# wadewilliamsw1234/Multi-level-Indoor-SLAM

Measured on AMD Instinct MI355X. Metric: keyframes gated/sec (VPR+kNN+LightGlue verify), higher is better.
Workload: dtype bf16

## Files before the change

include/mlgate.h:

```cpp
#ifndef MLGATE_H
#define MLGATE_H

#include <stddef.h>
#include <stdint.h>

#ifdef __cplusplus
extern "C" {
#endif

#define MLG_OK 0
#define MLG_EINVAL (-1)
#define MLG_EHIP (-2)
#define MLG_ENOMEM (-3)

#define MLG_VIT_DEPTH 12
#define MLG_VIT_EMBED 768
#define MLG_VIT_PATCH_K 768

#define MLG_ABI_VERSION 3
#define MLG_STRUCT_INIT(T) {(uint32_t)sizeof(T), (uint32_t)MLG_ABI_VERSION}
int mlg_abi_version(void);
const char* mlg_strerror(int status);

typedef struct mlg_vit_block {
    const float *norm1_w, *norm1_b;
    const uint16_t* qkv_w;
    const float* qkv_b;
    const uint16_t* proj_w;
    const float *proj_b, *ls1;
    const float *norm2_w, *norm2_b;
    const uint16_t* fc1_w;
    const float* fc1_b;
    const uint16_t* fc2_w;
    const float *fc2_b, *ls2;
} mlg_vit_block;

typedef struct mlg_vit_weights {
    uint32_t struct_size, abi_version;
    const uint16_t* patch_w;
    const float* patch_b;
    const float* cls;
    const float* pos;
    mlg_vit_block blocks[MLG_VIT_DEPTH];
    const float *norm_w, *norm_b;
    int packing;
} mlg_vit_weights;

#define MLG_VIT_POOL_MEAN 1
#define MLG_VIT_KEEP_CHANNELS 2
#define MLG_VIT_SPLIT 4

size_t mlg_vit_workspace_bytes(int batch, int image_size);

int mlg_vit_forward(const mlg_vit_weights* w, const uint8_t* frames, int batch, int H, int W, int C,
                    long frame_stride, int image_size, int flags, void* workspace, size_t workspace_bytes,
                    float* desc_out, float* local_out, void* stream);

typedef struct mlg_salad_weights {
    uint32_t struct_size, abi_version;
    const uint16_t* w1;
    const float* b1;
    const uint16_t* w2;
    const float* b2;
    const float *wt1, *bt1, *wt2, *bt2;
    float dust_bin;
} mlg_salad_weights;

#define MLG_SALAD_DIM 8448

size_t mlg_salad_workspace_bytes(int batch, int image_size);

int mlg_salad_forward(const mlg_vit_weights* w, const mlg_salad_weights* sw, const uint8_t* frames, int batch,
                      int H, int W, int C, long frame_stride, int image_size, void* workspace,
                      size_t workspace_bytes, float* desc_out, void* stream);

size_t mlg_knn_workspace_bytes(int N, int D, int Q);
size_t mlg_knn_workspace_bytes_k(int N, int D, int Q, int k, int query);
int mlg_knn_gate(const float* desc, int N, int D, const double* t, const int64_t* floor, const uint8_t* has_floor,
                 double min_gap, float thr, int k, int gating, int q0, int Q, void* workspace,
                 size_t workspace_bytes, int32_t* idx, float* sim, uint8_t* valid, int32_t* count,
                 unsigned long long* totals, void* stream);

int mlg_knn_query(const float* db, int N, int D, const float* qdesc, int Q, const double* t_db,
                  const double* t_query, double min_gap, int k, void* workspace, size_t workspace_bytes,
                  int32_t* idx, float* sim, int32_t* count, void* stream);

int mlg_row_normalize_f32(const float* X, float* Xn, int N, int D, float* norms_or_null, void* stream);
int mlg_similarity(const float* A, int Q, const float* B, int N, int D, float* S, void* stream);

size_t mlg_xcorr_workspace_bytes(int n1, int n2, int D);
int mlg_xcorr_score(const float* q, int n1, const float* m, int n2, int D, void* workspace, size_t workspace_bytes,
                    float* score, void* stream);

size_t mlg_xcorr_batch_workspace_bytes(int F, int L, int D, int P);
int mlg_xcorr_batch(const float* feats, int F, int L, int D, const int32_t* query, const int32_t* cand, int P,
                    void* workspace, size_t workspace_bytes, float* scores, void* stream);

int mlg_op_gemm_f32out(const uint16_t* A, const uint16_t* W, float* C, int M, int N, int K, void* stream);
int mlg_set_gemm_variant(int variant);
int mlg_op_gemm_f32out_variant(int variant, const uint16_t* A, const uint16_t* W, float* C, int M, int N, int K,
                               void* stream);
int mlg_op_gemm_bias_gelu(const uint16_t* A, const uint16_t* W, const float* bias, uint16_t* C, int M, int N,
                          int K, void* stream);
int mlg_op_gemm_residual(const uint16_t* A, const uint16_t* W, const float* bias, const float* gamma, float* X,
                         int M, int N, int K, void* stream);
int mlg_op_layernorm_bf16(const float* X, const float* g, const float* b, uint16_t* Y, int M, void* stream);
int mlg_op_attention(const uint16_t* Q, const uint16_t* K, const uint16_t* Vt, uint16_t* O, int B, int T, int Tpad,
                     int32_t* task_ws, void* stream);
int mlg_op_attention_varlen(const uint16_t* Q, const uint16_t* K, const uint16_t* Vt, uint16_t* O, int ldo, int Npad,
                            int heads, const int32_t* tasks, const int32_t* out_off, int ntasks, int max_q,
                            void* stream);
int mlg_op_lg_ffn(const uint16_t* ctx, float* X, uint16_t* xcopy, int ldc, int M, const uint16_t* Wout,
                  const float* bout, const uint16_t* Wf1, const float* bf1, const float* ln_g, const float* ln_b,
                  const uint16_t* Wf2, const float* bf2, void* stream);
int mlg_op_lg_proj(int self_block, const uint16_t* xcopy, int ldx, const uint16_t* W, const float* bias,
                   const float* ecos, const float* esin, const uint8_t* live, uint16_t* Q, uint16_t* K, uint16_t* Vt,
                   int Npad, void* stream);
int mlg_op_conv2d_nhwc(const uint16_t* in, const uint16_t* zero16, int B, int H, int W, int C, int k, int s,
                       const uint16_t* Wt, const float* bias, float* out, int N, void* stream);
int mlg_op_preprocess_patches(const uint8_t* frames, int B, int H, int W, int C, long frame_stride, int S,
                              uint16_t* patches, void* stream);

size_t mlg_plane_ransac_workspace_bytes(int S, int iterations);
int mlg_plane_ransac(const float* pts, const int32_t* offsets, int S, int iterations, uint64_t seed, double threshold,
                     void* workspace, size_t workspace_bytes, double* plane, double* ratio, int32_t* inliers,
                     void* stream);

size_t mlg_proximity_workspace_bytes(int N, int nrows);
int mlg_proximity_count(const double* pos, const int64_t* floor, int N, int row0, int nrows, double radius,
                        int min_gap, int strict, void* workspace, size_t workspace_bytes, long long* totals,
                        void* stream);
int mlg_proximity_emit(const double* pos, const int64_t* floor, int N, int row0, int nrows, double radius,
                       int min_gap, int strict, const void* workspace, size_t workspace_bytes, int32_t* pairs,
                       double* dist, uint8_t* valid, void* stream);

typedef struct mlg_rn_block {
    const uint16_t* w1; const float* b1;
    const uint16_t* w2; const float* b2;
    const uint16_t* w3; const float* b3;
    const uint16_t* wd; const float* bd;
} mlg_rn_block;
typedef struct mlg_rn_weights {
    uint32_t struct_size, abi_version;
    const float* stem_w;
    const float* stem_b;
    mlg_rn_block blocks[16];
} mlg_rn_weights;
size_t mlg_resnet50_workspace_bytes(int B, int H, int W);
int mlg_resnet50_forward(const mlg_rn_weights* w, const uint8_t* frames, int B, int H, int W, int C,
                         long frame_stride, int descriptor_dim, void* workspace, size_t workspace_bytes,
                         float* desc, void* stream);
int mlg_op_pillow_resize_224(const uint8_t* frames, int B, int H, int W, int C, long frame_stride, void* workspace,
                             size_t workspace_bytes, uint8_t* out, void* stream);

typedef struct mlg_mixvpr_weights {
    uint32_t struct_size, abi_version;
    const float* stem_w;
    const float* stem_b;
    mlg_rn_block blocks[13];
    const uint16_t* mix_w;
    const float* mix_p;
    const float* row_w;
    const float* chan_w;
    const float* chan_b;
    const float* row_s;
    const float* row_b;
} mlg_mixvpr_weights;
#define MLG_MIXVPR_DIM 4096
#define MLG_MIXVPR_SIZE 320
size_t mlg_mixvpr_workspace_bytes(int B, int H, int W);
int mlg_mixvpr_forward(const mlg_mixvpr_weights* w, const uint8_t* frames, int B, int H, int W, int C,
                       long frame_stride, void* workspace, size_t workspace_bytes, float* desc, void* stream);
int mlg_op_mixvpr_preprocess(const uint8_t* frames, int B, int H, int W, int C, long frame_stride, float* out,
                             void* stream);
int mlg_op_mixvpr_head(const mlg_mixvpr_weights* w, const float* features, int B, float* desc, void* stream);

typedef struct mlg_sp_weights {
    uint32_t struct_size, abi_version;
    const float* conv1a_w;
    const float* conv1a_b;
    const uint16_t* w[11];
    const float* b[11];
} mlg_sp_weights;
size_t mlg_superpoint_workspace_bytes(int B, int H, int W);
int mlg_superpoint(const mlg_sp_weights* w, const uint8_t* frames, int B, int H, int W, int C, long frame_stride,
                   float detection_threshold, int max_keypoints, int nms_radius, int remove_borders, void* workspace,
                   size_t workspace_bytes, float* keypoints, float* scores, float* descriptors,
                   uint16_t* descriptors_bf16, int32_t* counts, void* stream);
// ... 146 lines not shown
```

multi-level-indoor-slam_amd/csrc/abi.cpp:

```cpp
#include <hip/hip_runtime.h>

#include <math.h>

#include <mutex>
#include <vector>

#include "../../include/mlgate.h"
#include <cstddef>

#include "kernels.h"

namespace {

constexpr int PATCH = 14;

inline size_t align_up(size_t v, size_t a = 256) { return (v + a - 1) / a * a; }

struct VitGeom {
    int B, S, grid, P, T, Tpad;
    explicit VitGeom(int b, int s) : B(b), S(s), grid(s / PATCH), P(grid * grid), T(grid * grid + 1) {
        Tpad = (T + 63) / 64 * 64;
    }
};

// ... 452 lines not shown
size_t mlg_superglue_workspace_bytes(int P, int kmax) { return mlg_superglue_ws_bytes(P, kmax); }

int mlg_superglue(const mlg_sg_weights* w, const float* keypoints, const float* scores, const float* descriptors,
                  const int32_t* counts, int F, int kmax, int W, int H, const int32_t* pair_a, const int32_t* pair_b,
                  int P, int sinkhorn_iterations, float match_threshold, void* workspace, size_t workspace_bytes,
                  int32_t* matches, float* match_scores, int32_t* num_matches, void* stream) {
    if (!mlg_head_ok(w, MLG_ABI_VERSION) || !keypoints || !scores || !descriptors || !counts || !pair_a || !pair_b ||
        !workspace || !matches || !match_scores || !num_matches || F <= 0 || P <= 0 || W <= 0 || H <= 0)
        return MLG_EINVAL;
    for (int p = 0; p < P; ++p)
        if (pair_a[p] < 0 || pair_a[p] >= F || pair_b[p] < 0 || pair_b[p] >= F) return MLG_EINVAL;
    const mlg_sg_weights_i& wi = *reinterpret_cast<const mlg_sg_weights_i*>(&w->kenc_w);
    return mlg_superglue_run(wi, keypoints, scores, descriptors, counts, kmax, W, H, pair_a, pair_b, P,
                             sinkhorn_iterations, match_threshold, workspace, workspace_bytes, matches, match_scores,
                             num_matches, (hipStream_t)stream);
}

size_t mlg_ransac_workspace_bytes(int P, long S_total, int hypotheses) {
    return mlg_ransac_ws_bytes(P, S_total, hypotheses);
}

int mlg_ransac_epipolar(const float* kp1, const float* kp2, const int32_t* offsets, int P, long S_total,
                        const double* K, int k_stride, double threshold, int hypotheses, uint64_t seed,
                        void* workspace, size_t workspace_bytes, double* model, uint8_t* mask, int32_t* inliers,
                        double* pose, int32_t* status, void* stream) {
    if (!offsets || !workspace || !model || !inliers || !status || (S_total > 0 && (!kp1 || !kp2 || !mask)))
        return MLG_EINVAL;
    if (K && k_stride != 0 && k_stride != 9) return MLG_EINVAL;
    return mlg_ransac_run(kp1, kp2, offsets, P, S_total, K, k_stride, threshold, hypotheses, seed, workspace,
                          workspace_bytes, model, mask, inliers, pose, status, (hipStream_t)stream);
}

int mlg_recover_pose(const float* kp1, const float* kp2, const int32_t* offsets, int P, const double* K,
                     int k_stride, const double* E, const uint8_t* mask, double* pose, void* stream) {
    if (!kp1 || !kp2 || !offsets || !K || !E || !mask || !pose) return MLG_EINVAL;
    if (k_stride != 0 && k_stride != 9) return MLG_EINVAL;
    return mlg_recover_pose_run(kp1, kp2, offsets, P, K, k_stride, E, mask, pose, (hipStream_t)stream);
}

size_t mlg_xcorr_workspace_bytes(int n1, int n2, int D) {
    if (n1 <= 0 || n2 <= 0 || D <= 0) return 0;
    return align_up((size_t)n1 * D * 4) + align_up((size_t)n2 * D * 4) + align_up((size_t)n1 * n2 * 4);
}

int mlg_xcorr_score(const float* q, int n1, const float* m, int n2, int D, void* workspace, size_t workspace_bytes,
                    float* score, void* stream) {
    if (!q || !m || !workspace || !score || n1 <= 0 || n2 <= 0 || D <= 0) return MLG_EINVAL;
    if (mlg_xcorr_workspace_bytes(n1, n2, D) > workspace_bytes) return MLG_ENOMEM;
    hipStream_t s = (hipStream_t)stream;
    float* qn = (float*)workspace;
    float* mn = (float*)((char*)workspace + align_up((size_t)n1 * D * 4));
    float* C = (float*)((char*)mn + align_up((size_t)n2 * D * 4));
    TRY(mlg_row_normalize(q, qn, n1, D, nullptr, s));
    TRY(mlg_row_normalize(m, mn, n2, D, nullptr, s));
    TRY(mlg_similarity_f32(qn, n1, mn, n2, D, C, n2, s));
    TRY(mlg_xcorr_reduce(C, n1, n2, score, s));
    return MLG_OK;
}

size_t mlg_xcorr_batch_workspace_bytes(int F, int L, int D, int P) { return mlg_xcorr_batch_ws_bytes(F, L, D, P); }

int mlg_xcorr_batch(const float* feats, int F, int L, int D, const int32_t* query, const int32_t* cand, int P,
                    void* workspace, size_t workspace_bytes, float* scores, void* stream) {
    return mlg_xcorr_batch_run(feats, F, L, D, query, cand, P, workspace, workspace_bytes, scores,
                               (hipStream_t)stream);
}

int mlg_op_gemm_f32out(const uint16_t* A, const uint16_t* W, float* C, int M, int N, int K, void* stream) {
    return mlg_gemm_f32out(A, W, C, M, N, K, (hipStream_t)stream);
}
int mlg_op_gemm_f32out_variant(int variant, const uint16_t* A, const uint16_t* W, float* C, int M, int N, int K,
                               void* stream) {
    return mlg_gemm_f32out_variant(variant, A, W, C, M, N, K, (hipStream_t)stream);
}
int mlg_set_gemm_variant(int variant) { return mlg_gemm_set_variant(variant); }
int mlg_op_gemm_bias_gelu(const uint16_t* A, const uint16_t* W, const float* bias, uint16_t* C, int M, int N,
                          int K, void* stream) {
    return mlg_gemm_bias_gelu_bf16(A, W, bias, C, M, N, K, (hipStream_t)stream);
}
int mlg_op_gemm_residual(const uint16_t* A, const uint16_t* W, const float* bias, const float* gamma, float* X,
                         int M, int N, int K, void* stream) {
    return mlg_gemm_residual(A, W, bias, gamma, X, M, N, K, (hipStream_t)stream);
}
int mlg_op_layernorm_bf16(const float* X, const float* g, const float* b, uint16_t* Y, int M, void* stream) {
    return mlg_layernorm_bf16(X, g, b, Y, M, (hipStream_t)stream);
}
int mlg_op_attention(const uint16_t* Q, const uint16_t* K, const uint16_t* Vt, uint16_t* O, int B, int T, int Tpad,
                     int32_t* task_ws, void* stream) {
    return mlg_attention(Q, K, Vt, O, B, T, Tpad, task_ws, (hipStream_t)stream);
}
int mlg_op_attention_varlen(const uint16_t* Q, const uint16_t* K, const uint16_t* Vt, uint16_t* O, int ldo, int Npad,
                            int heads, const int32_t* tasks, const int32_t* out_off, int ntasks, int max_q,
                            void* stream) {
    return mlg_attention_varlen(Q, K, Vt, O, ldo, Npad, heads, reinterpret_cast<const int4*>(tasks), out_off, ntasks,
                                max_q, (hipStream_t)stream);
}
int mlg_op_lg_ffn(const uint16_t* ctx, float* X, uint16_t* xcopy, int ldc, int M, const uint16_t* Wout,
                  const float* bout, const uint16_t* Wf1, const float* bf1, const float* ln_g, const float* ln_b,
                  const uint16_t* Wf2, const float* bf2, void* stream) {
    mlg_lg_block_i w{};
    w.Wout = Wout; w.bout = bout; w.Wf1 = Wf1; w.bf1 = bf1; w.ln_g = ln_g; w.ln_b = ln_b; w.Wf2 = Wf2; w.bf2 = bf2;
    return mlg_lg_ffn(ctx, X, xcopy, ldc, M, w, (hipStream_t)stream);
}
int mlg_op_lg_proj(int self_block, const uint16_t* xcopy, int ldx, const uint16_t* W, const float* bias,
                   const float* ecos, const float* esin, const uint8_t* live, uint16_t* Q, uint16_t* K, uint16_t* Vt,
                   int Npad, void* stream) {
    (void)esin;
    return mlg_lg_proj(self_block != 0, xcopy, ldx, W, bias, ecos, live, Q, K, Vt, Npad, (hipStream_t)stream);
}
int mlg_op_conv2d_nhwc(const uint16_t* in, const uint16_t* zero16, int B, int H, int W, int C, int k, int s,
                       const uint16_t* Wt, const float* bias, float* out, int N, void* stream) {
    return mlg_conv_implicit(in, zero16, B, H, W, C, k, s, Wt, bias, nullptr, 0, out, N, nullptr, 0, 0, N, N,
                             (hipStream_t)stream);
}
int mlg_op_preprocess_patches(const uint8_t* frames, int B, int H, int W, int C, long frame_stride, int S,
                              uint16_t* patches, void* stream) {
    return mlg_preprocess_patches(frames, B, H, W, C, frame_stride, S, MLG_VIT_PATCH_K, 1, patches,
                                  (hipStream_t)stream);
}

int mlg_prof_enable(int slot_mask) {
    std::lock_guard<std::mutex> lk(g_prof.mu);
    if (slot_mask && g_prof.pool.empty()) {
        g_prof.pool.resize(PROF_POOL);
        for (auto& e : g_prof.pool)
            if (hipEventCreate(&e) != hipSuccess) return MLG_EHIP;
    }
    g_prof.mask = (unsigned)slot_mask & ((1u << MLG_PROF_SLOTS) - 1);
    return MLG_OK;
}

int mlg_prof_reset(void) {
    std::lock_guard<std::mutex> lk(g_prof.mu);
    prof_collect();
    for (int i = 0; i < MLG_PROF_SLOTS; ++i) {
        g_prof.total[i] = 0;
        g_prof.work[i] = 0;
        g_prof.count[i] = 0;
    }
    return MLG_OK;
}

int mlg_prof_read(int slot, double* total_ms, long* launches) {
    if (slot < 0 || slot >= MLG_PROF_SLOTS || !total_ms || !launches) return MLG_EINVAL;
    std::lock_guard<std::mutex> lk(g_prof.mu);
    prof_collect();
    *total_ms = g_prof.total[slot];
    *launches = g_prof.count[slot];
    return MLG_OK;
}

int mlg_prof_read_work(int slot, double* flops) {
    if (slot < 0 || slot >= MLG_PROF_SLOTS || !flops) return MLG_EINVAL;
    std::lock_guard<std::mutex> lk(g_prof.mu);
    prof_collect();
    *flops = g_prof.work[slot];
    return MLG_OK;
}

}
```

multi-level-indoor-slam_amd/csrc/gemm_bf16.hip:

```cpp
#include <stdlib.h>

#include <type_traits>

#include "common.h"
#include "kernels.h"

namespace {

constexpr int BM = 128, BN = 128, BK = 64;
constexpr int TILE_BYTES = BM * BK * 2;

__device__ __forceinline__ int swz_off(int row, int chunk) {
    return row * (BK * 2) + ((chunk ^ ((row >> 1) & 7)) << 4);
}

struct EpiF32 {
    float* C; int ldc;
    __device__ void operator()(int m, int n, const f32x4& v) const {
        *reinterpret_cast<float4*>(C + (size_t)m * ldc + n) = make_float4(v[0], v[1], v[2], v[3]);
    }
};

struct EpiBiasF32 {
    float* C; int ldc; const float* bias;
// ... 679 lines not shown
    const bf16_t* sa = a_base(walk.tile);
    const bf16_t* sb = b_base(walk.tile);
    a_offsets(walk.tile, oa);
#define D256_DMA(ST, OA, SA, SB, t)                                                                        \
    {                                                                                                      \
        const unsigned b_ = lds_addr(ST);                                                                  \
        const bf16_t* sa_ = (SA) + (t) * BK;                                                               \
        const bf16_t* sb_ = (SB) + (t) * BK;                                                               \
        _Pragma("unroll") for (int i = 0; i < NA; ++i) dma16s((OA)[i], sa_, b_ + da + i * 1024);           \
        _Pragma("unroll") for (int i = 0; i < NB; ++i) dma16s(ob[i], sb_, b_ + db + i * 1024);             \
    }
#define D256_COMPUTE(ST)                                                                                   \
    _Pragma("unroll") for (int s = 0; s < 2; ++s) {                                                        \
        bf16x8 af[8], wf[4];                                                                               \
        const int ch = s * 4 + (lane >> 4);                                                                \
        _Pragma("unroll") for (int i = 0; i < 4; ++i) {                                                    \
            const int row = wn * 64 + i * 16 + (lane & 15);                                                \
            wf[i] = *reinterpret_cast<const bf16x8*>((ST) + A_BYTES + soff<64>(row, ch));                  \
        }                                                                                                  \
        _Pragma("unroll") for (int j = 0; j < 8; ++j) {                                                    \
            const int row = wm * 128 + j * 16 + (lane & 15);                                               \
            af[j] = *reinterpret_cast<const bf16x8*>((ST) + soff<64>(row, ch));                            \
        }                                                                                                  \
        _Pragma("unroll") for (int j = 0; j < 8; ++j) _Pragma("unroll") for (int i = 0; i < 4; ++i)        \
            acc[i][j] = __builtin_amdgcn_mfma_f32_16x16x32_bf16(wf[i], af[j], acc[i][j], 0, 0, 0);         \
    }

    D256_DMA(st0, oa, sa, sb, 0);
    __builtin_amdgcn_s_waitcnt(0xF70);
    __builtin_amdgcn_s_barrier();
    for (; walk.tile < walk.end; walk.tile += walk.step) {
        const int tile = walk.tile, next = walk.next(tile);
        unsigned na[NA];
        a_offsets(next, na);
        const bf16_t* nsa = a_base(next);
        const bf16_t* nsb = b_base(next);
        const int kn = next != tile ? 0 : nk - 1;
        f32x4 acc[4][8];
        zero_acc(acc);
        for (int t = 0; t < nk; t += 2) {
            D256_DMA(st1, oa, sa, sb, t + 1);
            D256_COMPUTE(st0);
            __builtin_amdgcn_s_waitcnt(0xF70);
            __builtin_amdgcn_s_barrier();
            if (t + 2 < nk) {
                D256_DMA(st0, oa, sa, sb, t + 2);
            } else {
                D256_DMA(st0, na, nsa, nsb, kn);
            }
            D256_COMPUTE(st1);
            __builtin_amdgcn_s_waitcnt(0xF70);
            __builtin_amdgcn_s_barrier();
        }
        const int mt = tile / nN, m0 = mt * TM, n0 = (tile - mt * nN) * TN;
        if constexpr (row_staged<Epi>::value) {
            gemm256_rows_epilogue<TM / 2, STAGE / 8>(epi, acc, st1 + wave * (STAGE / 8), m0 + wm * 128, n0 + wn * 64,
                                                     M, lane);
            __syncthreads();
        } else {
            frag_epilogue(epi, acc, m0 + wm * 128, n0 + wn * 64, M, lane);
        }
#pragma unroll
        for (int i = 0; i < NA; ++i) oa[i] = na[i];
        sa = nsa;
        sb = nsb;
    }
    __builtin_amdgcn_s_waitcnt(0xF70);
#undef D256_COMPUTE
#undef D256_DMA
}

template <class E, class = void>
struct staged_of { static constexpr int value = 0; };
template <class E>
struct staged_of<E, std::void_t<decltype(E::STAGED)>> { static constexpr int value = E::STAGED; };

template <class Epi>
__global__ __launch_bounds__(512, 1) void k_gemm256s(const bf16_t* __restrict__ A, const bf16_t* __restrict__ W,
                                                    int M, int N, int K0, int lda, int ldw, Epi epi, int nb,
                                                    long sA, long sW) {
    constexpr int BK = 32, TM = 256, TN = 256;
    constexpr int PLANE = TM * BK * 2;
    constexpr int STAGE = 4 * PLANE;
    __shared__ __attribute__((aligned(16))) char st0[STAGE];
    __shared__ __attribute__((aligned(16))) char st1[STAGE];
    constexpr int STG = staged_of<Epi>::value;
    __shared__ size_t skey[STG == 1 ? 8 : 1][32];
    const int tid = threadIdx.x, lane = tid & 63, wave = tid >> 6;
    const int nN = N / TN, nM = (M + TM - 1) / TM, nMN = nN * nM;
    TileWalk walk(nb * nMN);
    if (walk.done()) return;

    const DmaLane<BK> dl(lane);
    const int wm = wave & 1, wn = wave >> 1;
    const int nk = K0 / BK;
    const int drow = 2 * wave * 1024;
    unsigned ob[2];
#pragma unroll
    for (int i = 0; i < 2; ++i) {
        const int row = dl.row(2 * wave + i);
        ob[i] = (unsigned)(row * ldw + dl.chunk(row)) * 2u;
    }
    auto a_offsets = [&](int t, unsigned (&o)[2]) { lane_offsets(dl, wave, lda, ((t % nMN) / nN) * TM, M, o); };
    auto a_base = [&](int t) { return A + (t / nMN) * sA + (size_t)(((t % nMN) / nN) * TM) * lda; };
    auto b_base = [&](int t) { return W + (t / nMN) * sW + (size_t)((t % nN) * TN) * ldw; };
    unsigned oa[2];
    const bf16_t* sa = a_base(walk.tile);
    const bf16_t* sb = b_base(walk.tile);
    a_offsets(walk.tile, oa);
#define S256_DMA(ST, OA, SA, SB, t)                                                                        \
    {                                                                                                      \
        const unsigned b_ = lds_addr(ST) + drow;                                                           \
        const bf16_t* ah_ = (SA) + (t) * BK;                                                               \
        const bf16_t* wh_ = (SB) + (t) * BK;                                                               \
        _Pragma("unroll") for (int i = 0; i < 2; ++i) {                                                    \
            dma16s((OA)[i], ah_, b_ + i * 1024);                                                           \
            dma16s((OA)[i], ah_ + K0, b_ + PLANE + i * 1024);                                              \
            dma16s(ob[i], wh_, b_ + 2 * PLANE + i * 1024);                                                 \
            dma16s(ob[i], wh_ + K0, b_ + 3 * PLANE + i * 1024);                                            \
        }                                                                                                  \
    }
#define S256_COMPUTE(ST)                                                                                   \
    {                                                                                                      \
        bf16x8 af[8], wh[4], wl[4];                                                                        \
        const int ch = lane >> 4;                                                                          \
        _Pragma("unroll") for (int i = 0; i < 4; ++i) {                                                    \
            const int row = wn * 64 + i * 16 + (lane & 15);                                                \
            wh[i] = frag<BK>((ST) + 2 * PLANE, row, ch);                                                   \
            wl[i] = frag<BK>((ST) + 3 * PLANE, row, ch);                                                   \
        }                                                                                                  \
        _Pragma("unroll") for (int j = 0; j < 8; ++j)                                                      \
            af[j] = frag<BK>((ST), wm * 128 + j * 16 + (lane & 15), ch);                                   \
        __builtin_amdgcn_s_setprio(1);                                                                     \
        _Pragma("unroll") for (int j = 0; j < 8; ++j) _Pragma("unroll") for (int i = 0; i < 4; ++i) {      \
            acc[i][j] = __builtin_amdgcn_mfma_f32_16x16x32_bf16(wh[i], af[j], acc[i][j], 0, 0, 0);         \
            acc[i][j] = __builtin_amdgcn_mfma_f32_16x16x32_bf16(wl[i], af[j], acc[i][j], 0, 0, 0);         \
        }                                                                                                  \
        __builtin_amdgcn_s_setprio(0);                                                                     \
        _Pragma("unroll") for (int j = 0; j < 8; ++j)                                                      \
            af[j] = frag<BK>((ST) + PLANE, wm * 128 + j * 16 + (lane & 15), ch);                           \
        __builtin_amdgcn_s_setprio(1);                                                                     \
        _Pragma("unroll") for (int j = 0; j < 8; ++j) _Pragma("unroll") for (int i = 0; i < 4; ++i)        \
            acc[i][j] = __builtin_amdgcn_mfma_f32_16x16x32_bf16(wh[i], af[j], acc[i][j], 0, 0, 0);         \
        __builtin_amdgcn_s_setprio(0);                                                                     \
    }

    S256_DMA(st0, oa, sa, sb, 0);
    __builtin_amdgcn_s_waitcnt(0xF70);
    __builtin_amdgcn_s_barrier();
    for (; walk.tile < walk.end; walk.tile += walk.step) {
        const int tile = walk.tile, next = walk.next(tile);
        unsigned na[2];
        a_offsets(next, na);
        const bf16_t* nsa = a_base(next);
        const bf16_t* nsb = b_base(next);
        const int kn = next != tile ? 0 : nk - 1;
        f32x4 acc[4][8];
        zero_acc(acc);
        for (int t = 0; t < nk; t += 2) {
            S256_DMA(st1, oa, sa, sb, t + 1);
            S256_COMPUTE(st0);
            __builtin_amdgcn_s_waitcnt(0xF70);
            __builtin_amdgcn_s_barrier();
            if (t + 2 < nk) {
                S256_DMA(st0, oa, sa, sb, t + 2);
            } else {
                S256_DMA(st0, na, nsa, nsb, kn);
            }
            S256_COMPUTE(st1);
            __builtin_amdgcn_s_waitcnt(0xF70);
            __builtin_amdgcn_s_barrier();
        }
        const int tz = tile / nMN, lt = tile - tz * nMN, mz = tz * M;
        const int mt = lt / nN, m0 = mt * TM, n0 = (lt - mt * nN) * TN;
        auto epilogue = [&](auto check) {
            constexpr bool CHECK = decltype(check)::value;
            typename Epi::Col cols[4];
            typename Epi::Row rows[8];
#pragma unroll
            for (int i = 0; i < 4; ++i) cols[i] = epi.col(n0 + wn * 64 + i * 16 + (lane >> 4) * 4);
#pragma unroll
            for (int j = 0; j < 8; ++j) {
                const int m = m0 + wm * 128 + j * 16 + (lane & 15);
                rows[j] = epi.row(CHECK ? min(m, M - 1) : m);
            }
#pragma unroll
            for (int i = 0; i < 4; ++i) {
                const int n = n0 + wn * 64 + i * 16 + (lane >> 4) * 4;
                typename Epi::Pre pre[8];
#pragma unroll
                for (int j = 0; j < 8; ++j) {
                    const int m = m0 + wm * 128 + j * 16 + (lane & 15);
                    pre[j] = epi.pre(CHECK ? min(m, M - 1) : m, n, cols[i], rows[j]);
                }
#pragma unroll
                for (int j = 0; j < 8; ++j) {
                    const int m = m0 + wm * 128 + j * 16 + (lane & 15);
                    if (!CHECK || m < M) epi.apply(m, n, acc[i][j], cols[i], rows[j], pre[j]);
                }
            }
        };
        if constexpr (STG == 1) {
            const int nw = n0 + wn * 64;
            if (epi.staged_wave(nw)) {
                char* img = st1 + wave * 8192;
                typename Epi::Col cols[4];
#pragma unroll
                for (int i = 0; i < 4; ++i) cols[i] = epi.col(nw + i * 16 + (lane >> 4) * 4);
#pragma unroll
                for (int p = 0; p < 4; ++p) {
#pragma unroll
                    for (int jj = 0; jj < 2; ++jj) {
                        const int j = 2 * p + jj, r = jj * 16 + (lane & 15);
                        if ((lane >> 4) == 0) {
                            const int m = m0 + wm * 128 + j * 16 + (lane & 15);
                            skey[wave][r] = epi.row(min(m, M - 1)).key;
                        }
#pragma unroll
                        for (int i = 0; i < 4; ++i) {
                            uint2 h, l;
                            epi.stage2(acc[i][j], cols[i], h, l);
                            const int ch = 2 * i + ((lane >> 5) & 1);
                            const int o = r * 128 + ((ch ^ (r & 7)) << 4) + 8 * (((lane >> 4) ^ (r >> 3)) & 1);
                            *reinterpret_cast<uint2*>(img + o) = h;
                            *reinterpret_cast<uint2*>(img + 4096 + o) = l;
                        }
                    }
                    __builtin_amdgcn_s_waitcnt(0xc07f);
                    __builtin_amdgcn_wave_barrier();
#pragma unroll
                    for (int it = 0; it < 8; ++it) {
                        const int L = it * 64 + lane, q = L >> 8, r = (L >> 3) & 31, ch = L & 7;
                        const int m = m0 + wm * 128 + p * 32 + r;
                        uint4 d = *reinterpret_cast<const uint4*>(img + q * 4096 + r * 128 + ((ch ^ (r & 7)) << 4));
                        if ((r >> 3) & 1) d = make_uint4(d.z, d.w, d.x, d.y);
                        if (m < M) epi.put(m, nw + ch * 8, q, skey[wave][r], d);
                    }
                    __builtin_amdgcn_s_waitcnt(0xc07f);
                    __builtin_amdgcn_wave_barrier();
                }
            } else if (m0 + TM <= M) {
                epilogue(std::false_type{});
            } else {
                epilogue(std::true_type{});
            }
            __syncthreads();
        } else if constexpr (STG == 2) {
            const int nw = n0 + wn * 64;
            char* img = st1 + wave * 8192;
            typename Epi::Col cols[4];
#pragma unroll
            for (int i = 0; i < 4; ++i) cols[i] = epi.col(nw + i * 16 + (lane >> 4) * 4);
#pragma unroll
            for (int p = 0; p < 4; ++p) {
#pragma unroll
                for (int jj = 0; jj < 2; ++jj) {
                    const int j = 2 * p + jj, r = jj * 16 + (lane & 15);
#pragma unroll
                    for (int i = 0; i < 4; ++i) {
                        const int ch = 4 * i + (lane >> 4);
                        *reinterpret_cast<float4*>(img + r * 256 + ((ch ^ (r & 15)) << 4)) =
                            epi.stage4(acc[i][j], cols[i]);
                    }
                }
                __builtin_amdgcn_s_waitcnt(0xc07f);
                __builtin_amdgcn_wave_barrier();
                float4 xv[8];
#pragma unroll
                for (int it = 0; it < 8; ++it) {
                    const int L = it * 64 + lane, r = L >> 4, ch = L & 15;
                    xv[it] = epi.load4(mz + min(m0 + wm * 128 + p * 32 + r, M - 1), nw + ch * 4);
                }
#pragma unroll
                for (int it = 0; it < 8; ++it) {
                    const int L = it * 64 + lane, r = L >> 4, ch = L & 15;
                    const int m = m0 + wm * 128 + p * 32 + r;
                    const float4 y = *reinterpret_cast<const float4*>(img + r * 256 + ((ch ^ (r & 15)) << 4));
                    if (m < M) epi.put4(mz + m, nw + ch * 4, xv[it], y);
                }
                __builtin_amdgcn_s_waitcnt(0xc07f);
                __builtin_amdgcn_wave_barrier();
            }
            __syncthreads();
        } else {
            if (m0 + TM <= M) epilogue(std::false_type{});
            else epilogue(std::true_type{});
        }
#pragma unroll
        for (int i = 0; i < 2; ++i) oa[i] = na[i];
        sa = nsa;
        sb = nsb;
    }
    __builtin_amdgcn_s_waitcnt(0xF70);
#undef S256_COMPUTE
#undef S256_DMA
}

template <class Epi>
__global__ __launch_bounds__(512, 2) void k_gemm256q(const bf16_t* __restrict__ A, const bf16_t* __restrict__ W,
                                                    int M, int N, int K, int lda, int ldw, Epi epi) {
    constexpr int BK = 32, TM = 256, TN = 256;
    constexpr int A_BYTES = TM * BK * 2, STAGE = (TM + TN) * BK * 2;
    constexpr int NA = 2, NB = 2;
    constexpr int WAIT2 = 0xF70 | (2 * (NA + NB));
    __shared__ __attribute__((aligned(16))) char ringbuf[4 * STAGE];
    const int tid = threadIdx.x, lane = tid & 63, wave = tid >> 6;
    const int nN = N / TN, nM = (M + TM - 1) / TM;
    TileWalk walk(nN * nM);
    if (walk.done()) return;

    const DmaLane<BK> dl(lane);
    const int wm = wave & 1, wn = wave >> 1;
    const int da = NA * wave * 1024, db = A_BYTES + NB * wave * 1024;
    const int nk = K / BK;
    auto a_base = [&](int t) { return A + (size_t)((t / nN) * TM) * lda; };
    auto b_base = [&](int t) { return W + (size_t)((t % nN) * TN) * ldw; };
    int ftile = walk.tile, fk = 0, fslot = 0;
    unsigned ob[NB], foa[NA];
    lane_offsets(dl, wave, ldw, ob);
    lane_offsets(dl, wave, lda, (ftile / nN) * TM, M, foa);
    const bf16_t *fsa = a_base(ftile), *fsb = b_base(ftile);
    auto fetch_next = [&]() __attribute__((always_inline)) {
        const unsigned b_ = lds_addr(ringbuf + fslot * STAGE);
        const bf16_t* sa_ = fsa + fk * BK;
        const bf16_t* sb_ = fsb + fk * BK;
#pragma unroll
        for (int i = 0; i < NA; ++i) dma16s(foa[i], sa_, b_ + da + i * 1024);
#pragma unroll
        for (int i = 0; i < NB; ++i) dma16s(ob[i], sb_, b_ + db + i * 1024);
        fslot = (fslot + 1) & 3;
        if (++fk == nk) {
            const int nt = walk.next(ftile);
            if (nt != ftile) {
                fk = 0;
                ftile = nt;
                lane_offsets(dl, wave, lda, (ftile / nN) * TM, M, foa);
                fsa = a_base(ftile);
                fsb = b_base(ftile);
            } else {
                fk = nk - 1;
            }
        }
    };
    fetch_next();
    fetch_next();
    fetch_next();
    __builtin_amdgcn_s_waitcnt(WAIT2);
    __builtin_amdgcn_s_barrier();
    int cslot = 0;
    for (; walk.tile < walk.end; walk.tile += walk.step) {
        f32x4 acc[4][8];
        zero_acc(acc);
        for (int t = 0; t < nk; ++t) {
            fetch_next();
            const char* st = ringbuf + cslot * STAGE;
            mma_stage<BK, 8>(acc, st, st + A_BYTES, wm * 128, wn * 64, lane);
            cslot = (cslot + 1) & 3;
            __builtin_amdgcn_s_waitcnt(WAIT2);
            __builtin_amdgcn_s_barrier();
        }
        const int mt = walk.tile / nN, m0 = mt * TM, n0 = (walk.tile - mt * nN) * TN;
        frag_epilogue(epi, acc, m0 + wm * 128, n0 + wn * 64, M, lane);
    }
    __builtin_amdgcn_s_waitcnt(0xF70);
}
struct ConvGeom {
    const bf16_t* in; const bf16_t* zero; int H, W, C, kw, s, pad, Ho, Wo;
};

template <class Epi, int TN>
__global__ __launch_bounds__(512, 2) void k_conv256(ConvGeom g, const bf16_t* __restrict__ W, int M, int N, int K,
                                                    Epi epi) {
    constexpr int BK = 64, TM = 256;
    constexpr int WN = TN / 64, WM = 8 / WN, RM = TM / WM;
    constexpr int JM = RM / 16;
    constexpr int A_BYTES = TM * BK * 2, STAGE = (TM + TN) * BK * 2;
    constexpr int NA = 4, NB = TN / 64;
    __shared__ __attribute__((aligned(16))) char st0[STAGE];
// ... 251 lines not shown
```

multi-level-indoor-slam_amd/mlgate/_native.py:

```python
import ctypes
import os

_HERE = os.path.dirname(os.path.abspath(__file__))
LIB_PATH = os.path.join(_HERE, "libmlgate.so")
TORCH_LIB_PATH = os.path.join(_HERE, "libmlgate_torch.so")
OPS = ("vit_forward_into", "salad_forward", "knn_gate", "knn_query", "row_normalize", "similarity", "xcorr_score", "xcorr_batch",
       "superpoint",
       "lightglue", "ransac_epipolar", "recover_pose", "resnet50", "loftr_features", "loftr_pack_tails", "loftr_coarse_layer", "loftr_match", "superglue", "pillow_resize_224", "plane_ransac", "proximity",
       "jpeg_pixels", "mixvpr_forward", "mixvpr_head", "mixvpr_preprocess",
       "prof_enable", "prof_reset", "prof_read")


c_int, c_long, c_size_t, c_float, c_double, c_void_p = (
    ctypes.c_int, ctypes.c_long, ctypes.c_size_t, ctypes.c_float, ctypes.c_double, ctypes.c_void_p)

EXPORTS = {
    "mlg_abi_version": (c_int, []),
    "mlg_strerror": (ctypes.c_char_p, [c_int]),
    "mlg_vit_workspace_bytes": (c_size_t, [c_int, c_int]),
    "mlg_vit_forward": (c_int, [c_void_p, c_void_p, c_int, c_int, c_int, c_int, c_long, c_int, c_int, c_void_p,
                                c_size_t, c_void_p, c_void_p, c_void_p]),
    "mlg_salad_workspace_bytes": (c_size_t, [c_int, c_int]),
    "mlg_salad_forward": (c_int, [c_void_p, c_void_p, c_void_p, c_int, c_int, c_int, c_int, c_long, c_int,
                                  c_void_p, c_size_t, c_void_p, c_void_p]),
    "mlg_knn_workspace_bytes": (c_size_t, [c_int, c_int, c_int]),
    "mlg_knn_workspace_bytes_k": (c_size_t, [c_int, c_int, c_int, c_int, c_int]),
    "mlg_knn_gate": (c_int, [c_void_p, c_int, c_int, c_void_p, c_void_p, c_void_p, c_double, c_float, c_int,
                             c_int, c_int, c_int, c_void_p, c_size_t, c_void_p, c_void_p, c_void_p, c_void_p,
                             c_void_p, c_void_p]),
    "mlg_knn_query": (c_int, [c_void_p, c_int, c_int, c_void_p, c_int, c_void_p, c_void_p, c_double, c_int,
                              c_void_p, c_size_t, c_void_p, c_void_p, c_void_p, c_void_p]),
    "mlg_row_normalize_f32": (c_int, [c_void_p, c_void_p, c_int, c_int, c_void_p, c_void_p]),
    "mlg_similarity": (c_int, [c_void_p, c_int, c_void_p, c_int, c_int, c_void_p, c_void_p]),
    "mlg_xcorr_workspace_bytes": (c_size_t, [c_int, c_int, c_int]),
    "mlg_xcorr_score": (c_int, [c_void_p, c_int, c_void_p, c_int, c_int, c_void_p, c_size_t, c_void_p,
                                c_void_p]),
    "mlg_plane_ransac_workspace_bytes": (c_size_t, [c_int, c_int]),
    "mlg_plane_ransac": (c_int, [c_void_p, c_void_p, c_int, c_int, ctypes.c_uint64, c_double, c_void_p, c_size_t,
                                 c_void_p, c_void_p, c_void_p, c_void_p]),
    "mlg_proximity_workspace_bytes": (c_size_t, [c_int, c_int]),
    "mlg_proximity_count": (c_int, [c_void_p, c_void_p, c_int, c_int, c_int, c_double, c_int, c_int, c_void_p,
                                    c_size_t, c_void_p, c_void_p]),
    "mlg_proximity_emit": (c_int, [c_void_p, c_void_p, c_int, c_int, c_int, c_double, c_int, c_int, c_void_p,
                                   c_size_t, c_void_p, c_void_p, c_void_p, c_void_p]),
    "mlg_ransac_workspace_bytes": (c_size_t, [c_int, c_long, c_int]),
    "mlg_ransac_epipolar": (c_int, [c_void_p, c_void_p, c_void_p, c_int, c_long, c_void_p, c_int, c_double, c_int,
                                    ctypes.c_uint64, c_void_p, c_size_t, c_void_p, c_void_p, c_void_p, c_void_p,
                                    c_void_p, c_void_p]),
    "mlg_recover_pose": (c_int, [c_void_p, c_void_p, c_void_p, c_int, c_void_p, c_int, c_void_p, c_void_p, c_void_p,
                                 c_void_p]),
    "mlg_resnet50_workspace_bytes": (c_size_t, [c_int, c_int, c_int]),
    "mlg_resnet50_forward": (c_int, [c_void_p, c_void_p, c_int, c_int, c_int, c_int, c_long, c_int, c_void_p,
                                     c_size_t, c_void_p, c_void_p]),
    "mlg_op_pillow_resize_224": (c_int, [c_void_p, c_int, c_int, c_int, c_int, c_long, c_void_p, c_size_t,
                                         c_void_p, c_void_p]),
    "mlg_mixvpr_workspace_bytes": (c_size_t, [c_int, c_int, c_int]),
    "mlg_mixvpr_forward": (c_int, [c_void_p, c_void_p, c_int, c_int, c_int, c_int, c_long, c_void_p, c_size_t,
                                   c_void_p, c_void_p]),
    "mlg_op_mixvpr_preprocess": (c_int, [c_void_p, c_int, c_int, c_int, c_int, c_long, c_void_p, c_void_p]),
    "mlg_op_mixvpr_head": (c_int, [c_void_p, c_void_p, c_int, c_void_p, c_void_p]),
    "mlg_superpoint_workspace_bytes": (c_size_t, [c_int, c_int, c_int]),
    "mlg_superpoint": (c_int, [c_void_p, c_void_p, c_int, c_int, c_int, c_int, c_long, c_float, c_int, c_int, c_int,
                               c_void_p, c_size_t, c_void_p, c_void_p, c_void_p, c_void_p, c_void_p, c_void_p]),
    "mlg_lightglue_workspace_bytes": (c_size_t, [c_int, c_int]),
    "mlg_lightglue": (c_int, [c_void_p, c_void_p, c_void_p, c_void_p, c_int, c_int, c_void_p, c_void_p, c_int,
                              c_float, c_float, c_float, c_int, c_void_p, c_size_t, c_void_p, c_void_p, c_void_p,
                              c_void_p, c_void_p]),
    "mlg_op_gemm_f32out": (c_int, [c_void_p, c_void_p, c_void_p, c_int, c_int, c_int, c_void_p]),
    "mlg_op_gemm_f32out_variant": (c_int, [c_int, c_void_p, c_void_p, c_void_p, c_int, c_int, c_int, c_void_p]),
    "mlg_set_gemm_variant": (c_int, [c_int]),
    "mlg_set_loftr_similarity": (c_int, [c_int]),
    "mlg_op_gemm_bias_gelu": (c_int, [c_void_p, c_void_p, c_void_p, c_void_p, c_int, c_int, c_int, c_void_p]),
    "mlg_op_gemm_residual": (c_int, [c_void_p, c_void_p, c_void_p, c_void_p, c_void_p, c_int, c_int, c_int,
                                     c_void_p]),
    "mlg_op_layernorm_bf16": (c_int, [c_void_p, c_void_p, c_void_p, c_void_p, c_int, c_void_p]),
    "mlg_op_attention": (c_int, [c_void_p, c_void_p, c_void_p, c_void_p, c_int, c_int, c_int, c_void_p, c_void_p]),
    "mlg_op_attention_varlen": (c_int, [c_void_p, c_void_p, c_void_p, c_void_p, c_int, c_int, c_int, c_void_p,
                                        c_void_p, c_int, c_int, c_void_p]),
    "mlg_op_lg_ffn": (c_int, [c_void_p, c_void_p, c_void_p, c_int, c_int] + [c_void_p] * 8 + [c_void_p]),
    "mlg_op_lg_proj": (c_int, [c_int, c_void_p, c_int] + [c_void_p] * 8 + [c_int, c_void_p]),
    "mlg_op_conv2d_nhwc": (c_int, [c_void_p, c_void_p] + [c_int] * 6 + [c_void_p] * 3 + [c_int, c_void_p]),
    "mlg_op_preprocess_patches": (c_int, [c_void_p, c_int, c_int, c_int, c_int, c_long, c_int, c_void_p,
                                          c_void_p]),
    "mlg_prof_enable": (c_int, [c_int]),
    "mlg_prof_reset": (c_int, []),
    "mlg_prof_read": (c_int, [c_int, ctypes.POINTER(c_double), ctypes.POINTER(c_long)]),
    "mlg_prof_read_work": (c_int, [c_int, ctypes.POINTER(c_double)]),
    "mlg_lg_orient_matches": (c_int, [c_void_p] * 5 + [c_int, c_int] + [c_void_p] * 4),
    "mlg_xcorr_batch_workspace_bytes": (c_size_t, [c_int, c_int, c_int, c_int]),
    "mlg_xcorr_batch": (c_int, [c_void_p, c_int, c_int, c_int, c_void_p, c_void_p, c_int, c_void_p, c_size_t,
                                c_void_p, c_void_p]),
    "mlg_dbg_lg_trace_begin": (c_int, [c_void_p, c_size_t]),
    "mlg_dbg_lg_trace_end": (c_int, [c_void_p, c_void_p, c_int]),
    "mlg_dbg_fill_lds": (c_int, [ctypes.c_uint32, c_void_p, c_void_p]),
    "mlg_dbg_fill_regs": (c_int, [ctypes.c_uint32, c_void_p]),
    "mlg_dbg_ransac_poison_nsol": (c_int, [c_int, c_int]),
    "mlg_loftr_tails_bytes": (c_size_t, []),
    "mlg_loftr_pack_tails": (c_int, [c_void_p, c_void_p, c_void_p]),
    "mlg_op_loftr_coarse_layer_ws_bytes": (c_size_t, [c_int, c_int]),
    "mlg_op_loftr_coarse_layer": (c_int, [c_void_p, c_int, c_int, c_void_p, c_void_p, c_int, c_int, c_void_p, c_size_t,
                                          c_void_p]),
    "mlg_png_info": (c_int, [c_void_p, c_size_t, c_void_p, c_void_p, c_void_p, c_void_p]),
    "mlg_png_decode_bgr": (c_int, [c_void_p, c_void_p, c_int, c_void_p, c_int, c_int, c_int, c_void_p]),
    "mlg_png_load_bgr": (c_int, [c_void_p, c_int, c_void_p, c_int, c_int, c_int, c_void_p]),
    "mlg_jpeg_info": (c_int, [c_void_p, c_size_t, c_void_p]),
    "mlg_jpeg_coef_bytes": (c_size_t, [c_int, c_int]),
    "mlg_jpeg_coefs_decode": (c_int, [c_void_p, c_void_p, c_int, c_void_p, c_void_p, c_void_p, c_int, c_int, c_int,
                                      c_void_p]),
    "mlg_jpeg_coefs_load": (c_int, [c_void_p, c_int, c_void_p, c_void_p, c_void_p, c_int, c_int, c_int, c_void_p]),
    "mlg_jpeg_params_check": (c_int, [c_void_p, c_int, c_int, c_int, c_size_t]),
    "mlg_jpeg_pixels": (c_int, [c_void_p, c_void_p, c_void_p, c_int, c_int, c_int, c_void_p, c_void_p]),
}

_lib = None
_ops = None


class MlgateError(RuntimeError):
    pass


def lib():
    global _lib
    if _lib is None:
        if not os.path.exists(LIB_PATH):
            raise MlgateError(f"{LIB_PATH} is missing: build it with `python -c 'import __graft_entry__ as g; "
                              "g.build()'` (hipcc --offload-arch=gfx950)")
        L = ctypes.CDLL(LIB_PATH)
        for name, (res, args) in EXPORTS.items():
            fn = getattr(L, name)
            fn.restype = res
            fn.argtypes = args
        _lib = L
    return _lib


def ops():
    global _ops
    if _ops is None:
        import torch
        if not os.path.exists(TORCH_LIB_PATH):
            raise MlgateError(f"{TORCH_LIB_PATH} is missing: build it with `python -c 'import __graft_entry__ as g; "
                              "g.build()'`")
        lib()
        torch.ops.load_library(TORCH_LIB_PATH)
        _ops = torch.ops.mlgate
    return _ops


def lightglue_workspace_bytes(pairs, kmax):
    return int(lib().mlg_lightglue_workspace_bytes(int(pairs), int(kmax)))


def check(rc, what=""):
    if rc != 0:
        msg = lib().mlg_strerror(rc).decode()
        raise MlgateError(f"{what} failed: {msg} (status {rc})")
# ... 22 lines not shown
```

Before: 543.3.

## Restructure split-K256 GEMM main loop into finer DMA/MFMA phases with unified LDS

Rewrites the inner loop of the 256x256 split-precision GEMM kernel into four phases per stage. Each phase interleaves a slice of the next stage's async global-to-LDS loads with a subset of the MFMAs, using vmcnt waits and barriers between phases. The two LDS stages and the epilogue key buffer are merged into one array, and each wave now loads a fixed quarter of the A tile with row clamping. New ABI entry points for the split residual and GELU GEMMs are also exposed. The aim is to hide load latency behind compute, at the cost of more barriers and a more fragile schedule.

```diff
diff --git a/include/mlgate.h b/include/mlgate.h
--- a/include/mlgate.h
+++ b/include/mlgate.h
@@ -104,6 +104,10 @@
                           int K, void* stream);
 int mlg_op_gemm_residual(const uint16_t* A, const uint16_t* W, const float* bias, const float* gamma, float* X,
                          int M, int N, int K, void* stream);
+int mlg_op_gemm_residual_split(const uint16_t* A, const uint16_t* W, const float* bias, const float* gamma, float* X,
+                               int M, int N, int K0, void* stream);
+int mlg_op_gemm_bias_gelu_split(const uint16_t* A, const uint16_t* W, const float* bias, uint16_t* C, int M, int N,
+                                int K0, void* stream);
 int mlg_op_layernorm_bf16(const float* X, const float* g, const float* b, uint16_t* Y, int M, void* stream);
 int mlg_op_attention(const uint16_t* Q, const uint16_t* K, const uint16_t* Vt, uint16_t* O, int B, int T, int Tpad,
                      int32_t* task_ws, void* stream);
diff --git a/multi-level-indoor-slam_amd/csrc/abi.cpp b/multi-level-indoor-slam_amd/csrc/abi.cpp
--- a/multi-level-indoor-slam_amd/csrc/abi.cpp
+++ b/multi-level-indoor-slam_amd/csrc/abi.cpp
@@ -558,6 +558,14 @@
                          int M, int N, int K, void* stream) {
     return mlg_gemm_residual(A, W, bias, gamma, X, M, N, K, (hipStream_t)stream);
 }
+int mlg_op_gemm_residual_split(const uint16_t* A, const uint16_t* W, const float* bias, const float* gamma, float* X,
+                               int M, int N, int K0, void* stream) {
+    return mlg_gemm_residual_split(A, W, bias, gamma, X, M, N, K0, (hipStream_t)stream);
+}
+int mlg_op_gemm_bias_gelu_split(const uint16_t* A, const uint16_t* W, const float* bias, uint16_t* C, int M, int N,
+                                int K0, void* stream) {
+    return mlg_gemm_bias_gelu_split(A, W, bias, C, M, N, K0, (hipStream_t)stream);
+}
 int mlg_op_layernorm_bf16(const float* X, const float* g, const float* b, uint16_t* Y, int M, void* stream) {
     return mlg_layernorm_bf16(X, g, b, Y, M, (hipStream_t)stream);
 }
diff --git a/multi-level-indoor-slam_amd/csrc/gemm_bf16.hip b/multi-level-indoor-slam_amd/csrc/gemm_bf16.hip
--- a/multi-level-indoor-slam_amd/csrc/gemm_bf16.hip
+++ b/multi-level-indoor-slam_amd/csrc/gemm_bf16.hip
@@ -785,10 +785,10 @@
     constexpr int BK = 32, TM = 256, TN = 256;
     constexpr int PLANE = TM * BK * 2;
     constexpr int STAGE = 4 * PLANE;
-    __shared__ __attribute__((aligned(16))) char st0[STAGE];
-    __shared__ __attribute__((aligned(16))) char st1[STAGE];
     constexpr int STG = staged_of<Epi>::value;
-    __shared__ size_t skey[STG == 1 ? 8 : 1][32];
+    __shared__ __attribute__((aligned(16))) char lds[2 * STAGE + (STG == 1 ? 8 * 32 * sizeof(size_t) : 0)];
+    char* const st1 = lds + STAGE;
+    size_t (*const skey)[32] = reinterpret_cast<size_t (*)[32]>(lds + 2 * STAGE);
     const int tid = threadIdx.x, lane = tid & 63, wave = tid >> 6;
     const int nN = N / TN, nM = (M + TM - 1) / TM, nMN = nN * nM;
     TileWalk walk(nb * nMN);
@@ -797,83 +797,110 @@
     const DmaLane<BK> dl(lane);
     const int wm = wave & 1, wn = wave >> 1;
     const int nk = K0 / BK;
-    const int drow = 2 * wave * 1024;
+    const int uw = __builtin_amdgcn_readfirstlane(wave);
+    const int grp = uw >> 2;
+    const int apl = uw & 1;
+    const int agrp = ((uw >> 1) & 1) + 8 * (uw >> 2);
+    const unsigned lbase = lds_addr(lds);
+    const unsigned dw = lbase + 2 * PLANE + 2 * uw * 1024;
+    const unsigned da = lbase + apl * PLANE + agrp * 1024;
     unsigned ob[2];
 #pragma unroll
     for (int i = 0; i < 2; ++i) {
         const int row = dl.row(2 * wave + i);
         ob[i] = (unsigned)(row * ldw + dl.chunk(row)) * 2u;
     }
-    auto a_offsets = [&](int t, unsigned (&o)[2]) { lane_offsets(dl, wave, lda, ((t % nMN) / nN) * TM, M, o); };
-    auto a_base = [&](int t) { return A + (t / nMN) * sA + (size_t)(((t % nMN) / nN) * TM) * lda; };
+    const int arow = dl.row(((wave >> 1) & 1) + 8 * (wave >> 2));
+    const unsigned ach = (unsigned)dl.chunk(arow) * 2u;
+    auto a_rmax = [&](int t) { return M - 1 - ((t % nMN) / nN) * TM; };
+    auto a_base = [&](int t) { return A + (t / nMN) * sA + (size_t)(((t % nMN) / nN) * TM) * lda + apl * K0; };
     auto b_base = [&](int t) { return W + (t / nMN) * sW + (size_t)((t % nN) * TN) * ldw; };
-    unsigned oa[2];
     const bf16_t* sa = a_base(walk.tile);
     const bf16_t* sb = b_base(walk.tile);
-    a_offsets(walk.tile, oa);
-#define S256_DMA(ST, OA, SA, SB, t)                                                                        \
+    int rm = a_rmax(walk.tile);
+    unsigned fa[2], fw[2];
+    fa[0] = soff<BK>(wm * 128 + (lane & 15), lane >> 4);
+    fw[0] = soff<BK>(wn * 64 + (lane & 15), lane >> 4);
+    fa[1] = fa[0] + STAGE;
+    fw[1] = fw[0] + STAGE;
+    asm volatile("" : "+v"(fa[1]), "+v"(fw[1]));
+#define S256_DMA_W(ST, PB, i)                                                                              \
     {                                                                                                      \
-        const unsigned b_ = lds_addr(ST) + drow;                                                           \
-        const bf16_t* ah_ = (SA) + (t) * BK;                                                               \
-        const bf16_t* wh_ = (SB) + (t) * BK;                                                               \
-        _Pragma("unroll") for (int i = 0; i < 2; ++i) {                                                    \
-            dma16s((OA)[i], ah_, b_ + i * 1024);                                                           \
-            dma16s((OA)[i], ah_ + K0, b_ + PLANE + i * 1024);                                              \
-            dma16s(ob[i], wh_, b_ + 2 * PLANE + i * 1024);                                                 \
-            dma16s(ob[i], wh_ + K0, b_ + 3 * PLANE + i * 1024);                                            \
+        dma16s(ob[i], (PB), dw + (ST) + (i) * 1024);                                                       \
+        dma16s(ob[i], (PB) + K0, dw + (ST) + PLANE + (i) * 1024);                                          \
+    }
+#define S256_DMA_A(ST, RM, PA, q) \
+    dma16s((unsigned)(min(arow + 32 * (q), (RM)) * lda) * 2u + ach, (PA), da + (ST) + (q) * 2048)
+#define S256_VMCNT8 asm volatile("s_waitcnt vmcnt(8)" ::: "memory")
+#define S256_PHASE(ST, p, ...)                                                                             \
+    {                                                                                                      \
+        bf16x8 ah[2], al[2];                                                                               \
+        if ((p) == 0) {                                                                                    \
+            _Pragma("unroll") for (int i = 0; i < 4; ++i) {                                                \
+                wh[i] = *reinterpret_cast<const bf16x8*>(lds + fw[(ST) / STAGE] + 2 * PLANE + i * 1024);   \
+                wl[i] = *reinterpret_cast<const bf16x8*>(lds + fw[(ST) / STAGE] + 3 * PLANE + i * 1024);   \
+            }                                                                                              \
         }                                                                                                  \
-    }
-#define S256_COMPUTE(ST)                                                                                   \
-    {                                                                                                      \
-        bf16x8 af[8], wh[4], wl[4];                                                                        \
-        const int ch = lane >> 4;                                                                          \
-        _Pragma("unroll") for (int i = 0; i < 4; ++i) {                                                    \
-            const int row = wn * 64 + i * 16 + (lane & 15);                                                \
-            wh[i] = frag<BK>((ST) + 2 * PLANE, row, ch);                                                   \
-            wl[i] = frag<BK>((ST) + 3 * PLANE, row, ch);                                                   \
+        _Pragma("unroll") for (int jj = 0; jj < 2; ++jj) {                                                 \
+            ah[jj] = *reinterpret_cast<const bf16x8*>(lds + fa[(ST) / STAGE] + (2 * (p) + jj) * 1024);     \
+            al[jj] = *reinterpret_cast<const bf16x8*>(lds + fa[(ST) / STAGE] + PLANE + (2 * (p) + jj) * 1024); \
         }                                                                                                  \
-        _Pragma("unroll") for (int j = 0; j < 8; ++j)                                                      \
-            af[j] = frag<BK>((ST), wm * 128 + j * 16 + (lane & 15), ch);                                   \
+        __VA_ARGS__                                                                                        \
+        __builtin_amdgcn_s_barrier();                                                                      \
+        __builtin_amdgcn_s_waitcnt(0xc07f);                                                \
+        __builtin_amdgcn_sched_barrier(0);                                                                 \
         __builtin_amdgcn_s_setprio(1);                                                                     \
-        _Pragma("unroll") for (int j = 0; j < 8; ++j) _Pragma("unroll") for (int i = 0; i < 4; ++i) {      \
-            acc[i][j] = __builtin_amdgcn_mfma_f32_16x16x32_bf16(wh[i], af[j], acc[i][j], 0, 0, 0);         \
-            acc[i][j] = __builtin_amdgcn_mfma_f32_16x16x32_bf16(wl[i], af[j], acc[i][j], 0, 0, 0);         \
-        }                                                                                                  \
+        _Pragma("unroll") for (int jj = 0; jj < 2; ++jj) _Pragma("unroll") for (int i = 0; i < 4; ++i)     \
+            acc[i][2 * (p) + jj] =                                                                         \
+                __builtin_amdgcn_mfma_f32_16x16x32_bf16(wh[i], ah[jj], acc[i][2 * (p) + jj], 0, 0, 0);     \
+        _Pragma("unroll") for (int jj = 0; jj < 2; ++jj) _Pragma("unroll") for (int i = 0; i < 4; ++i)     \
+            acc[i][2 * (p) + jj] =                                                                         \
+                __builtin_amdgcn_mfma_f32_16x16x32_bf16(wl[i], ah[jj], acc[i][2 * (p) + jj], 0, 0, 0);     \
+        _Pragma("unroll") for (int jj = 0; jj < 2; ++jj) _Pragma("unroll") for (int i = 0; i < 4; ++i)     \
+            acc[i][2 * (p) + jj] =                                                                         \
+                __builtin_amdgcn_mfma_f32_16x16x32_bf16(wh[i], al[jj], acc[i][2 * (p) + jj], 0, 0, 0);     \
         __builtin_amdgcn_s_setprio(0);                                                                     \
-        _Pragma("unroll") for (int j = 0; j < 8; ++j)                                                      \
-            af[j] = frag<BK>((ST) + PLANE, wm * 128 + j * 16 + (lane & 15), ch);                           \
-        __builtin_amdgcn_s_setprio(1);                                                                     \
-        _Pragma("unroll") for (int j = 0; j < 8; ++j) _Pragma("unroll") for (int i = 0; i < 4; ++i)        \
-            acc[i][j] = __builtin_amdgcn_mfma_f32_16x16x32_bf16(wh[i], af[j], acc[i][j], 0, 0, 0);         \
-        __builtin_amdgcn_s_setprio(0);                                                                     \
-    }
-
-    S256_DMA(st0, oa, sa, sb, 0);
-    __builtin_amdgcn_s_waitcnt(0xF70);
-    __builtin_amdgcn_s_barrier();
+        __builtin_amdgcn_sched_barrier(0);                                                                 \
+        __builtin_amdgcn_s_barrier();                                                                      \
+    }
+
+    S256_DMA_W(0, sb, 0)
+    S256_DMA_W(0, sb, 1)
+#pragma unroll
+    for (int q = 0; q < 4; ++q) S256_DMA_A(0, rm, sa, q);
     for (; walk.tile < walk.end; walk.tile += walk.step) {
         const int tile = walk.tile, next = walk.next(tile);
-        unsigned na[2];
-        a_offsets(next, na);
+        const int nrm = a_rmax(next);
         const bf16_t* nsa = a_base(next);
         const bf16_t* nsb = b_base(next);
-        const int kn = next != tile ? 0 : nk - 1;
+        S256_DMA_W(STAGE, sb + BK, 0)
+        S256_DMA_W(STAGE, sb + BK, 1)
+        S256_DMA_A(STAGE, rm, sa + BK, 0);
+        S256_DMA_A(STAGE, rm, sa + BK, 1);
+        S256_VMCNT8;
+        __builtin_amdgcn_s_barrier();
+        if (grp) __builtin_amdgcn_s_barrier();
         f32x4 acc[4][8];
         zero_acc(acc);
         for (int t = 0; t < nk; t += 2) {
-            S256_DMA(st1, oa, sa, sb, t + 1);
-            S256_COMPUTE(st0);
-            __builtin_amdgcn_s_waitcnt(0xF70);
-            __builtin_amdgcn_s_barrier();
-            if (t + 2 < nk) {
-                S256_DMA(st0, oa, sa, sb, t + 2);
-            } else {
-                S256_DMA(st0, na, nsa, nsb, kn);
-            }
-            S256_COMPUTE(st1);
-            __builtin_amdgcn_s_waitcnt(0xF70);
-            __builtin_amdgcn_s_barrier();
-        }
+            const bool more = t + 2 < nk;
+            const bf16_t* a1 = sa + (t + 1) * BK;
+            const bf16_t* a2 = more ? sa + (t + 2) * BK : nsa;
+            const bf16_t* b2 = more ? sb + (t + 2) * BK : nsb;
+            const bf16_t* a3 = sa + (t + 3) * BK;
+            const bf16_t* b3 = sb + (t + 3) * BK;
+            const int r2 = more ? rm : nrm;
+            bf16x8 wh[4], wl[4];
+            S256_PHASE(0, 0, S256_DMA_A(STAGE, rm, a1, 2);)
+            S256_PHASE(0, 1, S256_DMA_A(STAGE, rm, a1, 3); S256_VMCNT8;)
+            S256_PHASE(0, 2, S256_DMA_W(0, b2, 0) S256_DMA_A(0, r2, a2, 0);)
+            S256_PHASE(0, 3, S256_DMA_W(0, b2, 1) S256_DMA_A(0, r2, a2, 1); S256_VMCNT8;)
+            S256_PHASE(STAGE, 0, S256_DMA_A(0, r2, a2, 2);)
+            S256_PHASE(STAGE, 1, S256_DMA_A(0, r2, a2, 3); S256_VMCNT8;)
+            S256_PHASE(STAGE, 2, if (more) { S256_DMA_W(STAGE, b3, 0) S256_DMA_A(STAGE, rm, a3, 0); })
+            S256_PHASE(STAGE, 3, if (more) { S256_DMA_W(STAGE, b3, 1) S256_DMA_A(STAGE, rm, a3, 1); S256_VMCNT8; })
+        }
+        if (!grp) __builtin_amdgcn_s_barrier();
         const int tz = tile / nMN, lt = tile - tz * nMN, mz = tz * M;
         const int mt = lt / nN, m0 = mt * TM, n0 = (lt - mt * nN) * TN;
         auto epilogue = [&](auto check) {
@@ -989,14 +1016,16 @@
             if (m0 + TM <= M) epilogue(std::false_type{});
             else epilogue(std::true_type{});
         }
-#pragma unroll
-        for (int i = 0; i < 2; ++i) oa[i] = na[i];
+        rm = nrm;
         sa = nsa;
         sb = nsb;
+        __builtin_amdgcn_s_waitcnt(0xF70);
     }
     __builtin_amdgcn_s_waitcnt(0xF70);
-#undef S256_COMPUTE
-#undef S256_DMA
+#undef S256_PHASE
+#undef S256_VMCNT8
+#undef S256_DMA_A
+#undef S256_DMA_W
 }
 
 template <class Epi>
diff --git a/multi-level-indoor-slam_amd/mlgate/_native.py b/multi-level-indoor-slam_amd/mlgate/_native.py
--- a/multi-level-indoor-slam_amd/mlgate/_native.py
+++ b/multi-level-indoor-slam_amd/mlgate/_native.py
@@ -73,6 +73,9 @@
     "mlg_op_gemm_bias_gelu": (c_int, [c_void_p, c_void_p, c_void_p, c_void_p, c_int, c_int, c_int, c_void_p]),
     "mlg_op_gemm_residual": (c_int, [c_void_p, c_void_p, c_void_p, c_void_p, c_void_p, c_int, c_int, c_int,
                                      c_void_p]),
+    "mlg_op_gemm_residual_split": (c_int, [c_void_p, c_void_p, c_void_p, c_void_p, c_void_p, c_int, c_int, c_int,
+                                           c_void_p]),
+    "mlg_op_gemm_bias_gelu_split": (c_int, [c_void_p, c_void_p, c_void_p, c_void_p, c_int, c_int, c_int, c_void_p]),
     "mlg_op_layernorm_bf16": (c_int, [c_void_p, c_void_p, c_void_p, c_void_p, c_int, c_void_p]),
     "mlg_op_attention": (c_int, [c_void_p, c_void_p, c_void_p, c_void_p, c_int, c_int, c_int, c_void_p, c_void_p]),
     "mlg_op_attention_varlen": (c_int, [c_void_p, c_void_p, c_void_p, c_void_p, c_int, c_int, c_int, c_void_p,
```

Measured after the change: 549.6 (median of 6 runs). 1.01x the previous value.
